# argmaxinc/DiffusionKit

Measured on NVIDIA H100. Metric: images/sec at 1024x1024 (FLUX.1-schnell 4-step), higher is better.
Workload: dtype bf16

## Files before the change

### diffusionkit_b200/build.py

```python
import os
import subprocess
import sys

HERE = os.path.dirname(os.path.abspath(__file__))
CSRC = os.path.join(HERE, "csrc")
LIB = os.path.join(HERE, "libdkb200.so")
SOURCES = ["api.cu", "gemm.cu", "conv_fused.cu", "attention.cu", "elementwise.cu", "text.cu"]
NVCC_FLAGS = [
    "-gencode", "arch=compute_90a,code=sm_90a",
    "-O3", "-lineinfo", "-std=c++17",
    "-Xcompiler", "-fPIC", "-Xcompiler", "-Wall",
    "--expt-relaxed-constexpr",
    "-Xptxas", "-v",
]


def _stale(obj, src):
    if not os.path.exists(obj):
        return True
    t = os.path.getmtime(obj)
    deps = [src] + [os.path.join(CSRC, f) for f in os.listdir(CSRC) if f.endswith((".cuh", ".h"))]
    deps.append(os.path.join(HERE, "..", "include", "dkb200.h"))
    return any(os.path.getmtime(d) > t for d in deps)


def build(force: bool = False, verbose: bool = False) -> str:
    nvcc = os.environ.get("NVCC", "/usr/local/cuda/bin/nvcc")
    objs = []
    procs = []
    for s in SOURCES:
        src = os.path.join(CSRC, s)
        if not os.path.exists(src):
            continue
        obj = os.path.join(CSRC, s.replace(".cu", ".o"))
        objs.append(obj)
        if force or _stale(obj, src):
            cmd = [nvcc, *NVCC_FLAGS, "-c", src, "-o", obj]
            procs.append((s, subprocess.Popen(cmd, stdout=subprocess.PIPE, stderr=subprocess.STDOUT, text=True)))
    failed = False
    for s, p in procs:
        out, _ = p.communicate()
        if p.returncode != 0:
            failed = True
            sys.stderr.write(f"[build] {s} FAILED\n{out}\n")
        elif verbose:
            sys.stderr.write(f"[build] {s}\n{out}\n")
    if failed:
        raise RuntimeError("nvcc failed")
    if procs or not os.path.exists(LIB):
        cmd = [nvcc, "-shared", "-Wno-deprecated-gpu-targets", "-o", LIB, *objs, "-lcudart", "-ldl"]
        subprocess.check_call(cmd)
    return LIB


if __name__ == "__main__":
    print(build(force="--force" in sys.argv, verbose="-v" in sys.argv))
```

### diffusionkit_b200/csrc/attention.cu

```cuda
#include "attention.cuh"

namespace dk {

constexpr int ATT_THREADS = 384;

template <typename T, int D>
__global__ void __launch_bounds__(ATT_THREADS, 1)
attention_fwd_kernel(const __grid_constant__ CUtensorMap tm, const AttParams p) {
  using H16 = Half16<T>;
  using Cfg = AttCfg<D>;
  constexpr int KS = Cfg::KS;
  extern __shared__ uint8_t smem_raw[];
  uint8_t* smem = smem_raw + ((1024u - (smem_u32(smem_raw) & 1023u)) & 1023u);
  uint8_t* sQ = smem + Cfg::OFF_Q;
  uint8_t* sK = smem + Cfg::OFF_K;
  uint8_t* sV = smem + Cfg::OFF_V;
  uint64_t* q_full = reinterpret_cast<uint64_t*>(smem + Cfg::OFF_BAR);
  uint64_t* k_full = q_full + 1;
  uint64_t* v_full = k_full + KS;
  uint64_t* kv_empty = v_full + KS;

  const int warp = threadIdx.x >> 5;
  const int lane = threadIdx.x & 31;
  const int wg = threadIdx.x >> 7;
  const int q0 = blockIdx.x * ATT_BQ;
  const int head = blockIdx.y;
  const int b = blockIdx.z;
  const int h = p.heads * D;
  const int row0 = b * p.S;
  const int nkv = (p.S + ATT_BKV - 1) / ATT_BKV;
  constexpr uint32_t TILE_BYTES = ATT_BKV * D * 2;

  if (threadIdx.x == 0) {
    tma_prefetch_desc(&tm);
    mbar_init(q_full, 1);
    for (int i = 0; i < KS; ++i) {
      mbar_init(&k_full[i], 1);
      mbar_init(&v_full[i], 1);
      mbar_init(&kv_empty[i], 8);
    }
    fence_barrier_init();
  }
  __syncthreads();

  if (wg == 0) {
    if (warp != 0) return;
    if (elect_one_sync()) {
      mbar_arrive_expect_tx(q_full, ATT_BQ * D * 2);
#pragma unroll
      for (int c = 0; c < D / 64; ++c) tma_load_2d(sQ + c * (ATT_BQ * 128), &tm, q_full, head * D + c * 64, row0 + q0);
    }
    __syncwarp();
    uint32_t stage = 0, phase = 0;
    for (int j = 0; j < nkv; ++j) {
      mbar_wait_warp(&kv_empty[stage], phase ^ 1);
      if (elect_one_sync()) {
        const int kr = row0 + j * ATT_BKV;
        mbar_arrive_expect_tx(&k_full[stage], TILE_BYTES);
#pragma unroll
        for (int c = 0; c < D / 64; ++c)
          tma_load_2d(sK + stage * TILE_BYTES + c * (ATT_BKV * 128), &tm, &k_full[stage], h + head * D + c * 64, kr);
        mbar_arrive_expect_tx(&v_full[stage], TILE_BYTES);
#pragma unroll
        for (int c = 0; c < D / 64; ++c)
          tma_load_2d(sV + stage * TILE_BYTES + c * (ATT_BKV * 128), &tm, &v_full[stage], 2 * h + head * D + c * 64, kr);
      }
      __syncwarp();
      if (++stage == KS) {
        stage = 0;
        phase ^= 1;
      }
    }
    return;
  }

  const int cw = wg - 1;
  const float sl2 = p.scale_log2;
  float o[D / 2];
#pragma unroll
  for (int i = 0; i < D / 2; ++i) o[i] = 0.f;
  float m_run[2] = {-INFINITY, -INFINITY};
  float l_run[2] = {0.f, 0.f};
  const int col0 = 2 * (lane & 3);

  mbar_wait(q_full, 0);
  const uint32_t q_base = smem_u32(sQ) + cw * 64 * 128;
  uint32_t stage = 0, phase = 0;
  for (int j = 0; j < nkv; ++j) {
    const int kv_valid = p.S - j * ATT_BKV;
    const uint32_t k_base = smem_u32(sK + stage * TILE_BYTES);
    const uint32_t v_base = smem_u32(sV + stage * TILE_BYTES);
    float s[ATT_BKV / 2];
    mbar_wait(&k_full[stage], phase);
    wgmma_fence();
#pragma unroll
    for (int kk = 0; kk < D / 16; ++kk) {
      const uint32_t koff = (kk >> 2) * (ATT_BKV * 128) + (kk & 3) * 32;
      Wgmma<ATT_BKV, H16::is_bf16, 0>::ss(s, make_smem_desc_sw128(q_base + (kk >> 2) * (ATT_BQ * 128) + (kk & 3) * 32, 16, 1024),
                                         make_smem_desc_sw128(k_base + koff, 16, 1024), kk != 0 ? 1u : 0u);
    }
    wgmma_commit();
    wgmma_wait<0>();
    reg_fence(s);

    float alpha[2];
#pragma unroll
    for (int i = 0; i < 2; ++i) {
      float mx = -INFINITY;
#pragma unroll
      for (int jj = 0; jj < ATT_BKV / 8; ++jj)
#pragma unroll
        for (int e = 0; e < 2; ++e) {
          float& v = s[4 * jj + 2 * i + e];
          if (kv_valid < ATT_BKV && 8 * jj + col0 + e >= kv_valid) v = -INFINITY;
          mx = fmaxf(mx, v);
        }
      mx = fmaxf(mx, __shfl_xor_sync(0xffffffffu, mx, 1));
      mx = fmaxf(mx, __shfl_xor_sync(0xffffffffu, mx, 2));
      const float m_new = fmaxf(m_run[i], mx * sl2);
      alpha[i] = ex2_approx(m_run[i] - m_new);
      m_run[i] = m_new;
      float ls = 0.f;
#pragma unroll
      for (int jj = 0; jj < ATT_BKV / 8; ++jj)
#pragma unroll
        for (int e = 0; e < 2; ++e) {
          float& v = s[4 * jj + 2 * i + e];
          v = ex2_approx(fmaf(v, sl2, -m_new));
          ls += v;
        }
      l_run[i] = l_run[i] * alpha[i] + ls;
    }
#pragma unroll
    for (int jj = 0; jj < D / 8; ++jj)
#pragma unroll
      for (int i = 0; i < 2; ++i) {
        o[4 * jj + 2 * i] *= alpha[i];
        o[4 * jj + 2 * i + 1] *= alpha[i];
      }
    uint32_t pa[ATT_BKV / 16][4];
#pragma unroll
    for (int kk = 0; kk < ATT_BKV / 16; ++kk) {
      pa[kk][0] = H16::pack(s[8 * kk + 0], s[8 * kk + 1]);
      pa[kk][1] = H16::pack(s[8 * kk + 2], s[8 * kk + 3]);
      pa[kk][2] = H16::pack(s[8 * kk + 4], s[8 * kk + 5]);
      pa[kk][3] = H16::pack(s[8 * kk + 6], s[8 * kk + 7]);
    }

    mbar_wait(&v_full[stage], phase);
    wgmma_fence();
#pragma unroll
    for (int kk = 0; kk < ATT_BKV / 16; ++kk)
      Wgmma<D, H16::is_bf16, 1>::rs(o, pa[kk], make_smem_desc_sw128(v_base + kk * 16 * 128, ATT_BKV * 128, 1024), 1u);
    wgmma_commit();
    wgmma_wait<0>();
    reg_fence(o);
    __syncwarp();
    if (lane == 0) mbar_arrive(&kv_empty[stage]);
    if (++stage == KS) {
      stage = 0;
      phase ^= 1;
    }
  }

#pragma unroll
  for (int i = 0; i < 2; ++i) {
    float l = l_run[i];
    l += __shfl_xor_sync(0xffffffffu, l, 1);
    l += __shfl_xor_sync(0xffffffffu, l, 2);
    const float inv_l = 1.0f / l;
    const int s_idx = q0 + cw * 64 + (warp & 3) * 16 + (lane >> 2) + 8 * i;
    if (s_idx >= p.S) continue;
    T* dst;
    if (s_idx < p.split)
      dst = reinterpret_cast<T*>(p.out0) + (static_cast<long long>(b) * p.split + s_idx) * p.ld0 + head * D;
    else
      dst = reinterpret_cast<T*>(p.out1) + (static_cast<long long>(b) * (p.S - p.split) + (s_idx - p.split)) * p.ld1 +
            head * D;
#pragma unroll
    for (int jj = 0; jj < D / 8; ++jj)
      *reinterpret_cast<uint32_t*>(dst + 8 * jj + col0) =
          H16::pack(o[4 * jj + 2 * i] * inv_l, o[4 * jj + 2 * i + 1] * inv_l);
  }
}

template <typename T, int D>
static int launch_attention(dk_ctx* ctx, const CUtensorMap& tm, const AttParams& p, cudaStream_t stream) {
  auto kern = attention_fwd_kernel<T, D>;
  static bool configured = false;
  if (!configured) {
    DK_CHECK_CUDA(cudaFuncSetAttribute(kern, cudaFuncAttributeMaxDynamicSharedMemorySize, AttCfg<D>::SMEM_BYTES));
    configured = true;
  }
  dim3 grid(dk_ceil_div(p.S, ATT_BQ), p.heads, p.B);
  kern<<<grid, ATT_THREADS, AttCfg<D>::SMEM_BYTES, stream>>>(tm, p);
  DK_LAUNCH_CHECK(ctx);
  return 0;
}

}

using namespace dk;

extern "C" int dk_attention_fwd(dk_ctx* ctx, int dtype, const void* qkv, int B, int S, int heads, int d, float scale,
                                int split, void* out0, long long ld0, void* out1, long long ld1, void* stream_) {
  DK_REQUIRE(ctx != nullptr, "dk_attention_fwd: null ctx");
  DkDeviceGuard dk_guard_(ctx);
  DK_REQUIRE(dtype == DK_BF16 || dtype == DK_FP16, "dk_attention_fwd: bad dtype %d", dtype);
  DK_REQUIRE(d == 64 || d == 128, "dk_attention_fwd: head dim %d unsupported (64 or 128)", d);
  DK_REQUIRE(B > 0 && S > 0 && heads > 0, "dk_attention_fwd: empty problem");
  DK_REQUIRE(split >= 0 && split <= S, "dk_attention_fwd: split %d outside [0, %d]", split, S);
  DK_REQUIRE(out0 != nullptr || split == 0, "dk_attention_fwd: out0 is NULL");
  DK_REQUIRE(out1 != nullptr || split == S, "dk_attention_fwd: out1 is NULL but split < S");
  DK_REQUIRE(ld0 % 8 == 0 && ld1 % 8 == 0, "dk_attention_fwd: output leading dims must be multiples of 8");
  DK_REQUIRE((reinterpret_cast<uintptr_t>(qkv) & 15u) == 0 && (reinterpret_cast<uintptr_t>(out0) & 15u) == 0 &&
                 (reinterpret_cast<uintptr_t>(out1) & 15u) == 0,
             "dk_attention_fwd: buffers must be 16-byte aligned");
  cudaStream_t stream = static_cast<cudaStream_t>(stream_);
  const int h = heads * d;
  CUtensorMap tm;
  const uint64_t dims[2] = {static_cast<uint64_t>(3 * h), static_cast<uint64_t>(B) * S};
  const uint64_t strides[1] = {static_cast<uint64_t>(3 * h) * 2};
  const uint32_t box[2] = {64, 128};
  if (int rc = dk_make_tmap_16b(ctx, &tm, qkv, 2, dims, strides, box)) return rc;
  AttParams p;
  p.B = B;
  p.S = S;
  p.heads = heads;
  p.split = split;
  p.scale_log2 = scale * 1.44269504088896341f;
  p.out0 = out0;
  p.ld0 = ld0;
  p.out1 = out1;
  p.ld1 = ld1;
  if (dtype == DK_BF16) {
    if (d == 128) return launch_attention<__nv_bfloat16, 128>(ctx, tm, p, stream);
    return launch_attention<__nv_bfloat16, 64>(ctx, tm, p, stream);
  }
  if (d == 128) return launch_attention<__half, 128>(ctx, tm, p, stream);
  return launch_attention<__half, 64>(ctx, tm, p, stream);
}
```

### diffusionkit_b200/csrc/common.cuh

```cuda
#pragma once

#include <cuda.h>
#include <cuda_bf16.h>
#include <cuda_fp16.h>
#include <cuda_runtime.h>
#include <stdint.h>
#include <stdio.h>

#include "wgmma.cuh"

namespace dk {

__device__ __forceinline__ uint32_t smem_u32(const void* p) {
  return static_cast<uint32_t>(__cvta_generic_to_shared(p));
}


#ifndef DK_WATCHDOG_CYCLES
#define DK_WATCHDOG_CYCLES (8000000000LL)
#endif

__device__ __forceinline__ void mbar_init(uint64_t* bar, uint32_t count) {
  asm volatile("mbarrier.init.shared::cta.b64 [%0], %1;" ::"r"(smem_u32(bar)), "r"(count) : "memory");
}
__device__ __forceinline__ void fence_barrier_init() {
  asm volatile("fence.mbarrier_init.release.cluster;" ::: "memory");
}
__device__ __forceinline__ void mbar_arrive(uint64_t* bar) {
  asm volatile("mbarrier.arrive.shared::cta.b64 _, [%0];" ::"r"(smem_u32(bar)) : "memory");
}
__device__ __forceinline__ void mbar_arrive_expect_tx(uint64_t* bar, uint32_t bytes) {
  asm volatile("mbarrier.arrive.expect_tx.shared::cta.b64 _, [%0], %1;" ::"r"(smem_u32(bar)), "r"(bytes)
               : "memory");
}
__device__ __forceinline__ uint32_t mbar_try_wait(uint64_t* bar, uint32_t parity) {
  uint32_t ok;
  asm volatile(
      "{\n\t.reg .pred p;\n\t"
      "mbarrier.try_wait.parity.shared::cta.b64 p, [%1], %2;\n\t"
      "selp.u32 %0, 1, 0, p;\n\t}"
      : "=r"(ok)
      : "r"(smem_u32(bar)), "r"(parity)
      : "memory");
  return ok;
}
#ifndef DK_WATCHDOG_SPINS
#define DK_WATCHDOG_SPINS (1u << 26)
#endif
static __device__ __noinline__ void mbar_watchdog_trap(uint64_t* bar, uint32_t parity) {
  printf("[dkb200] mbarrier watchdog: block (%d,%d,%d) thread %d bar@%u parity %u\n", blockIdx.x, blockIdx.y, blockIdx.z,
         threadIdx.x, smem_u32(bar), parity);
  __trap();
}
__device__ __forceinline__ void mbar_wait(uint64_t* bar, uint32_t parity) {
  if (mbar_try_wait(bar, parity)) return;
  uint32_t spins = 0;
  while (!mbar_try_wait(bar, parity)) {
    if (++spins == DK_WATCHDOG_SPINS) mbar_watchdog_trap(bar, parity);
  }
}

__device__ __forceinline__ void mbar_wait_nocall(uint64_t* bar, uint32_t parity) {
  uint32_t spins = 0;
  while (!mbar_try_wait(bar, parity)) {
    if (++spins == DK_WATCHDOG_SPINS) asm volatile("trap;");
  }
}

__device__ __forceinline__ void mbar_wait_warp(uint64_t* bar, uint32_t parity) {
  if ((threadIdx.x & 31) == 0) mbar_wait(bar, parity);
  __syncwarp();
}

__device__ __forceinline__ void st_shared_u32(uint32_t addr, uint32_t v) {
  asm volatile("st.shared.u32 [%0], %1;" ::"r"(addr), "r"(v));
}

__device__ __forceinline__ void fence_proxy_async_smem() {
  asm volatile("fence.proxy.async.shared::cta;" ::: "memory");
}

__device__ __forceinline__ void named_bar_sync(uint32_t id, uint32_t nthreads) {
  asm volatile("bar.sync %0, %1;" ::"r"(id), "r"(nthreads) : "memory");
}

__device__ __forceinline__ uint32_t cluster_ctarank() {
  uint32_t r;
  asm volatile("mov.u32 %0, %%cluster_ctarank;" : "=r"(r));
  return r;
}
__device__ __forceinline__ void cluster_sync() {
  asm volatile("barrier.cluster.arrive.release;\n\tbarrier.cluster.wait.acquire;" ::: "memory");
}
__device__ __forceinline__ void mbar_arrive_cluster(uint64_t* bar, uint32_t cta) {
  asm volatile(
      "{\n\t.reg .b32 ra;\n\t"
      "mapa.shared::cluster.u32 ra, %0, %1;\n\t"
      "mbarrier.arrive.shared::cluster.b64 _, [ra];\n\t}" ::"r"(smem_u32(bar)),
      "r"(cta)
      : "memory");
}

__device__ __forceinline__ void tma_prefetch_desc(const CUtensorMap* m) {
  asm volatile("prefetch.tensormap [%0];" ::"l"(reinterpret_cast<uint64_t>(m)) : "memory");
}
__device__ __forceinline__ void tma_load_2d(void* dst, const CUtensorMap* map, uint64_t* bar, int c0, int c1) {
  asm volatile(
      "cp.async.bulk.tensor.2d.shared::cluster.global.tile.mbarrier::complete_tx::bytes [%0], [%1, {%3, %4}], [%2];" ::
          "r"(smem_u32(dst)),
      "l"(reinterpret_cast<uint64_t>(map)), "r"(smem_u32(bar)), "r"(c0), "r"(c1)
      : "memory");
}
__device__ __forceinline__ void tma_load_2d_multicast(void* dst, const CUtensorMap* map, uint64_t* bar, int c0, int c1,
                                                      uint16_t cta_mask) {
  asm volatile(
      "cp.async.bulk.tensor.2d.shared::cluster.global.tile.mbarrier::complete_tx::bytes.multicast::cluster "
      "[%0], [%1, {%3, %4}], [%2], %5;" ::"r"(smem_u32(dst)),
      "l"(reinterpret_cast<uint64_t>(map)), "r"(smem_u32(bar)), "r"(c0), "r"(c1), "h"(cta_mask)
      : "memory");
}
__device__ __forceinline__ void tma_load_4d(void* dst, const CUtensorMap* map, uint64_t* bar, int c0, int c1, int c2,
                                            int c3) {
  asm volatile(
      "cp.async.bulk.tensor.4d.shared::cluster.global.tile.mbarrier::complete_tx::bytes [%0], [%1, {%3, %4, %5, %6}], "
      "[%2];" ::"r"(smem_u32(dst)),
      "l"(reinterpret_cast<uint64_t>(map)), "r"(smem_u32(bar)), "r"(c0), "r"(c1), "r"(c2), "r"(c3)
      : "memory");
}

__device__ __forceinline__ void wgmma_fence() { asm volatile("wgmma.fence.sync.aligned;" ::: "memory"); }
__device__ __forceinline__ void wgmma_commit() { asm volatile("wgmma.commit_group.sync.aligned;" ::: "memory"); }
template <int N>
__device__ __forceinline__ void wgmma_wait() {
  asm volatile("wgmma.wait_group.sync.aligned %0;" ::"n"(N) : "memory");
}
template <int N>
__device__ __forceinline__ void reg_fence(float (&d)[N]) {
#pragma unroll
  for (int i = 0; i < N; ++i) asm volatile("" : "+f"(d[i])::"memory");
}

template <int N>
__device__ __forceinline__ void setmaxnreg_inc() {
  asm volatile("setmaxnreg.inc.sync.aligned.u32 %0;" ::"n"(N));
}
template <int N>
__device__ __forceinline__ void setmaxnreg_dec() {
  asm volatile("setmaxnreg.dec.sync.aligned.u32 %0;" ::"n"(N));
}
__device__ __forceinline__ float ex2_approx(float x) {
  float y;
  asm("ex2.approx.ftz.f32 %0, %1;" : "=f"(y) : "f"(x));
  return y;
}

__device__ __forceinline__ uint64_t make_smem_desc_sw128(uint32_t smem_addr, uint32_t lbo_bytes, uint32_t sbo_bytes) {
  uint64_t d = 0;
  d |= static_cast<uint64_t>((smem_addr & 0x3FFFFu) >> 4);
  d |= static_cast<uint64_t>((lbo_bytes >> 4) & 0x3FFFu) << 16;
  d |= static_cast<uint64_t>((sbo_bytes >> 4) & 0x3FFFu) << 32;
  d |= static_cast<uint64_t>(1) << 62;
  return d;
}

__device__ __forceinline__ bool elect_one_sync() {
  uint32_t pred;
  asm volatile(
      "{\n\t.reg .pred p;\n\t"
      "elect.sync _|p, 0xffffffff;\n\t"
      "selp.u32 %0, 1, 0, p;\n\t}"
      : "=r"(pred));
  return pred != 0;
}

template <int N>
__device__ __forceinline__ void stage_acc_rows(float* stage, int ld, int row0, const float (&d)[N / 2]) {
  const int t = threadIdx.x & 127;
  const int r = row0 + (t >> 5) * 16 + ((t & 31) >> 2);
  const int c = 2 * (t & 3);
#pragma unroll
  for (int j = 0; j < N / 8; ++j)
#pragma unroll
    for (int i = 0; i < 2; ++i)
      *reinterpret_cast<float2*>(stage + (r + 8 * i) * ld + 8 * j + c) = make_float2(d[4 * j + 2 * i], d[4 * j + 2 * i + 1]);
}

template <typename T>
struct Half16;
template <>
struct Half16<__nv_bfloat16> {
  using T2 = __nv_bfloat162;
  static constexpr bool is_bf16 = true;
  __device__ static __forceinline__ float to_f(__nv_bfloat16 v) { return __bfloat162float(v); }
  __device__ static __forceinline__ __nv_bfloat16 from_f(float v) { return __float2bfloat16_rn(v); }
  __device__ static __forceinline__ uint32_t pack(float lo, float hi) {
    __nv_bfloat162 t = __floats2bfloat162_rn(lo, hi);
    return *reinterpret_cast<uint32_t*>(&t);
  }
  __device__ static __forceinline__ float2 unpack(uint32_t u) {
    __nv_bfloat162 t = *reinterpret_cast<__nv_bfloat162*>(&u);
    return __bfloat1622float2(t);
  }
};
template <>
struct Half16<__half> {
  using T2 = __half2;
  static constexpr bool is_bf16 = false;
  __device__ static __forceinline__ float to_f(__half v) { return __half2float(v); }
  __device__ static __forceinline__ __half from_f(float v) { return __float2half_rn(v); }
  __device__ static __forceinline__ uint32_t pack(float lo, float hi) {
    __half2 t = __floats2half2_rn(lo, hi);
    return *reinterpret_cast<uint32_t*>(&t);
  }
  __device__ static __forceinline__ float2 unpack(uint32_t u) {
    __half2 t = *reinterpret_cast<__half2*>(&u);
    return __half22float2(t);
  }
};

__device__ __forceinline__ float gelu_erf(float v) { return 0.5f * v * (1.0f + erff(v * 0.70710678118654752f)); }
__device__ __forceinline__ float silu_f(float v) {
  float e;
  asm("ex2.approx.ftz.f32 %0, %1;" : "=f"(e) : "f"(-1.4426950408889634f * v));
  return __fdividef(v, 1.0f + e);
}

__device__ __forceinline__ float quick_gelu_f(float v) {
  float e;
  asm("ex2.approx.ftz.f32 %0, %1;" : "=f"(e) : "f"(-1.702f * 1.4426950408889634f * v));
  return __fdividef(v, 1.0f + e);
}

__device__ __forceinline__ float warp_sum(float v) {
#pragma unroll
  for (int o = 16; o > 0; o >>= 1) v += __shfl_xor_sync(0xffffffffu, v, o);
  return v;
}
__device__ __forceinline__ float warp_max(float v) {
#pragma unroll
  for (int o = 16; o > 0; o >>= 1) v = fmaxf(v, __shfl_xor_sync(0xffffffffu, v, o));
  return v;
}

}
```

### diffusionkit_b200/csrc/conv_fused.cu

```cuda
#include <stdlib.h>

#include "common.cuh"
#include "host.h"

namespace dk {

constexpr int CF_TW = 128;
constexpr int CF_R = 2;
constexpr int CF_BN = 128;
constexpr int CF_HW = CF_TW + 2;
constexpr int CF_HR = CF_R + 2;
constexpr int CF_A_BYTES = CF_HR * CF_HW * 128;
constexpr int CF_B_BYTES = CF_BN * 64 * 2;
constexpr int CF_A_BUFS = 2;
constexpr int CF_B_STAGES = 4;
constexpr int CF_THREADS = 384;
constexpr int CF_STAGE_LD = CF_BN + 4;
constexpr int CF_STAT_BYTES = 8 * CF_R * 2 * 8 * 2 * 4;
constexpr int CF_OFF_B = CF_A_BUFS * CF_A_BYTES;
constexpr int CF_OFF_STAT = CF_OFF_B + CF_B_STAGES * CF_B_BYTES;
constexpr int CF_OFF_BAR = CF_OFF_STAT + CF_STAT_BYTES;
constexpr int CF_SMEM_BYTES = CF_OFF_BAR + 256 + 1024;
static_assert(CF_OFF_STAT >= CF_R * CF_TW * CF_STAGE_LD * 4, "conv_fused: the staging tile reuses the pipeline buffers");
static_assert(CF_SMEM_BYTES <= 232448, "conv_fused: shared memory budget");

struct ConvFParams {
  int B, H, W;
  int Cin, Cout;
  int up;
  int tiles_x, tiles_y;
  int n_tiles;
  const void* bias;
  const void* res;
  void* out;
  const float* gn_stats;
  const void* gamma;
  const void* beta;
  int G;
  int silu;
  float* out_partial;
  int out_G;
};

__device__ __forceinline__ float tanh_approx(float x) {
  float y;
  asm("tanh.approx.f32 %0, %1;" : "=f"(y) : "f"(x));
  return y;
}

struct CfItem {
  int b, ty, tx, phase, nt;
};
__device__ __forceinline__ void cf_decode(const ConvFParams& p, int item, CfItem& it) {
  const int phases = p.up ? 4 : 1;
  it.nt = item % p.n_tiles;
  item /= p.n_tiles;
  it.phase = item % phases;
  item /= phases;
  it.tx = item % p.tiles_x;
  item /= p.tiles_x;
  it.ty = item % p.tiles_y;
  it.b = item / p.tiles_y;
}

template <int N>
__device__ __forceinline__ void warp_multi_sum(float (&v)[N], int lane) {
  int off = 16;
#pragma unroll
  for (int n = N; n > 1; n >>= 1, off >>= 1) {
    const bool hi = (lane & off) != 0;
#pragma unroll
    for (int i = 0; i < n / 2; ++i) {
      const float keep = hi ? v[i + n / 2] : v[i];
      const float send = hi ? v[i] : v[i + n / 2];
      v[i] = keep + __shfl_xor_sync(0xffffffffu, send, off);
    }
  }
#pragma unroll
  for (; off > 0; off >>= 1) v[0] += __shfl_xor_sync(0xffffffffu, v[0], off);
}
template <int N>
__device__ __forceinline__ int warp_multi_index(int lane) {
  int idx = 0, off = 16;
#pragma unroll
  for (int n = N; n > 1; n >>= 1, off >>= 1) idx += (lane & off) ? n / 2 : 0;
  return idx;
}

template <int CPG>
__device__ __forceinline__ void cf_chunk_stats(const float (&v)[32], float* dst, int lane) {
  constexpr int NG = 32 / CPG;
  constexpr int N = 2 * NG;
  float a[N];
#pragma unroll
  for (int g = 0; g < NG; ++g) {
    float s = 0.f, q = 0.f;
#pragma unroll
    for (int c = 0; c < CPG; ++c) {
      const float t = v[g * CPG + c];
      s += t;
      q = fmaf(t, t, q);
    }
    a[g] = s;
    a[NG + g] = q;
  }
  warp_multi_sum<N>(a, lane);
  constexpr int LOW = 32 / N;
  if ((lane & (LOW - 1)) == 0) {
    const int idx = warp_multi_index<N>(lane);
    const int g = idx % NG, which = idx / NG;
    dst[g * 2 + which] = a[0];
  }
}

template <typename T>
__global__ void __launch_bounds__(CF_THREADS, 1)
conv_fused_kernel(const __grid_constant__ CUtensorMap tmX, const __grid_constant__ CUtensorMap tmW, const ConvFParams p) {
  using H16 = Half16<T>;
  extern __shared__ uint8_t smem_raw[];
  uint8_t* smem = smem_raw + ((1024u - (smem_u32(smem_raw) & 1023u)) & 1023u);
  uint8_t* sA = smem;
  uint8_t* sB = smem + CF_OFF_B;
  float* sstat = reinterpret_cast<float*>(smem + CF_OFF_STAT);
  uint64_t* bars = reinterpret_cast<uint64_t*>(smem + CF_OFF_BAR);
  uint64_t* a_land = bars;
  uint64_t* a_empty = a_land + CF_A_BUFS;
  uint64_t* b_full = a_empty + CF_A_BUFS;
  uint64_t* b_empty = b_full + CF_B_STAGES;

  const int warp = threadIdx.x >> 5;
  const int lane = threadIdx.x & 31;
  const int wg = threadIdx.x >> 7;
  const int cblocks = p.Cin / 64;
  const int ntaps = p.up ? 4 : 9;
  CfItem it;
  cf_decode(p, blockIdx.x, it);
  const int py = it.phase >> 1, px = it.phase & 1;
  const int y0 = it.ty * CF_R;
  const int x0 = it.tx * CF_TW;

  if (threadIdx.x == 0) {
    tma_prefetch_desc(&tmX);
    tma_prefetch_desc(&tmW);
    for (int i = 0; i < CF_A_BUFS; ++i) {
      mbar_init(&a_land[i], 1);
      mbar_init(&a_empty[i], 8);
    }
    for (int i = 0; i < CF_B_STAGES; ++i) {
      mbar_init(&b_full[i], 1);
      mbar_init(&b_empty[i], 8);
    }
    fence_barrier_init();
  }
  __syncthreads();

  if (wg == 0) {
    if (warp != 0) return;
    uint32_t bst = 0, bph = 0;
    uint32_t abuf = 0, aph = 0;
    const int w_row = it.phase * p.Cout + it.nt * CF_BN;
    for (int cb = 0; cb < cblocks; ++cb) {
      mbar_wait_warp(&a_empty[abuf], aph ^ 1);
      if (elect_one_sync()) {
        mbar_arrive_expect_tx(&a_land[abuf], CF_A_BYTES);
        tma_load_4d(sA + abuf * CF_A_BYTES, &tmX, &a_land[abuf], cb * 64, x0 - 1, y0 - 1, it.b);
      }
      __syncwarp();
      if (++abuf == CF_A_BUFS) {
        abuf = 0;
        aph ^= 1;
      }
      for (int tap = 0; tap < ntaps; ++tap) {
        mbar_wait_warp(&b_empty[bst], bph ^ 1);
        if (elect_one_sync()) {
          mbar_arrive_expect_tx(&b_full[bst], CF_B_BYTES);
          tma_load_2d(sB + bst * CF_B_BYTES, &tmW, &b_full[bst], tap * p.Cin + cb * 64, w_row);
        }
        __syncwarp();
        if (++bst == CF_B_STAGES) {
          bst = 0;
          bph ^= 1;
        }
      }
    }
    return;
  }

  const int rr = wg - 1;
  const int tid = threadIdx.x - 128;
  float acc0[CF_BN / 2], acc1[CF_BN / 2];
#pragma unroll
  for (int i = 0; i < CF_BN / 2; ++i) {
    acc0[i] = 0.f;
    acc1[i] = 0.f;
  }
  {
    constexpr int TT = 256;
    const int chunk = tid & 7;
    const int cpg = p.gn_stats != nullptr ? p.Cin / p.G : 1;
    uint32_t bst = 0, bph = 0, abuf = 0, aph = 0;
    for (int cb = 0; cb < cblocks; ++cb) {
      mbar_wait(&a_land[abuf], aph);
      if (p.gn_stats != nullptr) {
        float sc[8], sh[8];
        {
          const int c0 = cb * 64 + chunk * 8;
          const uint4 g4 = *reinterpret_cast<const uint4*>(reinterpret_cast<const T*>(p.gamma) + c0);
          const uint4 b4 = *reinterpret_cast<const uint4*>(reinterpret_cast<const T*>(p.beta) + c0);
          const uint32_t gw[4] = {g4.x, g4.y, g4.z, g4.w}, bw[4] = {b4.x, b4.y, b4.z, b4.w};
#pragma unroll
          for (int i = 0; i < 4; ++i) {
            const float2 gf = H16::unpack(gw[i]), bf = H16::unpack(bw[i]);
#pragma unroll
            for (int h2 = 0; h2 < 2; ++h2) {
              const int g = (c0 + 2 * i + h2) / cpg;
              const float mean = __ldg(p.gn_stats + (it.b * p.G + g) * 2), rstd = __ldg(p.gn_stats + (it.b * p.G + g) * 2 + 1);
              const float ga = h2 ? gf.y : gf.x, be = h2 ? bf.y : bf.x;
              sc[2 * i + h2] = rstd * ga;
              sh[2 * i + h2] = be - mean * rstd * ga;
            }
          }
        }
        const uint32_t base = smem_u32(sA) + abuf * CF_A_BYTES;
        const bool do_silu = p.silu != 0;
        auto in_image = [&](int q) {
          const int hr = q / CF_HW, hx = q - hr * CF_HW;
          const int gy = y0 - 1 + hr, gx = x0 - 1 + hx;
          return q < CF_HR * CF_HW && gy >= 0 && gy < p.H && gx >= 0 && gx < p.W;
        };
        auto xform = [&](uint32_t (&w)[4]) {
#pragma unroll
          for (int i = 0; i < 4; ++i) {
            const float2 f = H16::unpack(w[i]);
            float a = fmaf(f.x, sc[2 * i], sh[2 * i]);
            float b = fmaf(f.y, sc[2 * i + 1], sh[2 * i + 1]);
            if (do_silu) {
              const float ha = 0.5f * a, hb = 0.5f * b;
              a = fmaf(ha, tanh_approx(ha), ha);
              b = fmaf(hb, tanh_approx(hb), hb);
            }
            w[i] = H16::pack(a, b);
          }
        };
        for (int q0 = tid >> 3; q0 < CF_HR * CF_HW; q0 += 2 * (TT / 8)) {
          const int q1 = q0 + TT / 8;
          const bool ok0 = in_image(q0), ok1 = in_image(q1);
          const uint32_t addr0 = base + q0 * 128 + ((chunk ^ (q0 & 7)) << 4);
          const uint32_t addr1 = base + q1 * 128 + ((chunk ^ (q1 & 7)) << 4);
          uint32_t w0[4] = {0u, 0u, 0u, 0u}, w1[4] = {0u, 0u, 0u, 0u};
          if (ok0) asm volatile("ld.shared.v4.b32 {%0, %1, %2, %3}, [%4];" : "=r"(w0[0]), "=r"(w0[1]), "=r"(w0[2]), "=r"(w0[3]) : "r"(addr0));
          if (ok1) asm volatile("ld.shared.v4.b32 {%0, %1, %2, %3}, [%4];" : "=r"(w1[0]), "=r"(w1[1]), "=r"(w1[2]), "=r"(w1[3]) : "r"(addr1));
          xform(w0);
          xform(w1);
          if (ok0) asm volatile("st.shared.v4.b32 [%0], {%1, %2, %3, %4};" ::"r"(addr0), "r"(w0[0]), "r"(w0[1]), "r"(w0[2]), "r"(w0[3]) : "memory");
          if (ok1) asm volatile("st.shared.v4.b32 [%0], {%1, %2, %3, %4};" ::"r"(addr1), "r"(w1[0]), "r"(w1[1]), "r"(w1[2]), "r"(w1[3]) : "memory");
        }
        fence_proxy_async_smem();
        named_bar_sync(1, 256);
      }
      const uint32_t a_addr0 = smem_u32(sA) + abuf * CF_A_BYTES;
      uint32_t prev = 0;
      for (int tap = 0; tap < ntaps; ++tap) {
        const int dy = p.up ? ((tap >> 1) + py) : (tap / 3);
        const int dx = p.up ? ((tap & 1) + px) : (tap - (tap / 3) * 3);
        mbar_wait(&b_full[bst], bph);
        const uint32_t b_addr = smem_u32(sB) + bst * CF_B_BYTES;
        const uint32_t a_addr = a_addr0 + ((rr + dy) * CF_HW + dx) * 128;
        wgmma_fence();
#pragma unroll
        for (int k = 0; k < 4; ++k) {
          const uint32_t acc_on = (cb | tap | k) != 0 ? 1u : 0u;
          const uint64_t db = make_smem_desc_sw128(b_addr + k * 32, 16, 1024);
          Wgmma<CF_BN, H16::is_bf16, 0>::ss(acc0, make_smem_desc_sw128(a_addr + k * 32, 16, 1024), db, acc_on);
          Wgmma<CF_BN, H16::is_bf16, 0>::ss(acc1, make_smem_desc_sw128(a_addr + 64 * 128 + k * 32, 16, 1024), db, acc_on);
        }
        wgmma_commit();
        if (tap > 0) {
          wgmma_wait<1>();
          if (lane == 0) mbar_arrive(&b_empty[prev]);
        }
        prev = bst;
        if (++bst == CF_B_STAGES) {
          bst = 0;
          bph ^= 1;
        }
      }
      wgmma_wait<0>();
      if (lane == 0) {
        mbar_arrive(&b_empty[prev]);
        mbar_arrive(&a_empty[abuf]);
      }
      if (++abuf == CF_A_BUFS) {
        abuf = 0;
        aph ^= 1;
      }
    }
    reg_fence(acc0);
    reg_fence(acc1);
  }

  float* stg = reinterpret_cast<float*>(smem);
  named_bar_sync(1, 256);
  stage_acc_rows<CF_BN>(stg, CF_STAGE_LD, rr * CF_TW, acc0);
  stage_acc_rows<CF_BN>(stg, CF_STAGE_LD, rr * CF_TW + 64, acc1);
  named_bar_sync(1, 256);

  const int ew = warp - 4;
  const int quarter = ew & 3;
  const int half = ew >> 2;
  const int xl = quarter * 32 + lane;
  const T* bias = reinterpret_cast<const T*>(p.bias);
  const T* res = reinterpret_cast<const T*>(p.res);
  T* out = reinterpret_cast<T*>(p.out);
  const int Hout = p.up ? 2 * p.H : p.H, Wout = p.up ? 2 * p.W : p.W;
  const int cpg_out = p.out_partial != nullptr ? p.Cout / p.out_G : 8;
  const int slots = (Hout * Wout) / CF_TW;
  const int x = x0 + xl;
  const int n_base = it.nt * CF_BN + half * 64;
  float* st_my = sstat + (ew * CF_R) * (2 * 8 * 2);
#pragma unroll 1
  for (int r2 = 0; r2 < CF_R; ++r2) {
    const int oy = p.up ? 2 * (y0 + r2) + py : (y0 + r2);
    const int ox = p.up ? 2 * x + px : x;
    const long long orow = (static_cast<long long>(it.b) * Hout + oy) * Wout + ox;
#pragma unroll
    for (int ch = 0; ch < 2; ++ch) {
      const float* src = stg + (r2 * CF_TW + xl) * CF_STAGE_LD + half * 64 + ch * 32;
      const int n0 = n_base + ch * 32;
      float v[32];
#pragma unroll
      for (int j = 0; j < 4; ++j) {
        if (n0 + j * 8 >= p.Cout) {
#pragma unroll
          for (int i = 0; i < 8; ++i) v[j * 8 + i] = 0.f;
          continue;
        }
        const float4 a4 = *reinterpret_cast<const float4*>(src + j * 8);
        const float4 b4f = *reinterpret_cast<const float4*>(src + j * 8 + 4);
        const float r[8] = {a4.x, a4.y, a4.z, a4.w, b4f.x, b4f.y, b4f.z, b4f.w};
        float bv[8] = {0.f, 0.f, 0.f, 0.f, 0.f, 0.f, 0.f, 0.f};
        if (bias != nullptr) {
          const uint4 b4 = *reinterpret_cast<const uint4*>(bias + n0 + j * 8);
          const uint32_t bw[4] = {b4.x, b4.y, b4.z, b4.w};
#pragma unroll
          for (int i = 0; i < 4; ++i) {
            const float2 f = H16::unpack(bw[i]);
            bv[2 * i] = f.x;
            bv[2 * i + 1] = f.y;
          }
        }
        float rv[8] = {0.f, 0.f, 0.f, 0.f, 0.f, 0.f, 0.f, 0.f};
        if (res != nullptr) {
          const uint4 r4 = *reinterpret_cast<const uint4*>(res + orow * p.Cout + n0 + j * 8);
          const uint32_t rw[4] = {r4.x, r4.y, r4.z, r4.w};
#pragma unroll
          for (int i = 0; i < 4; ++i) {
            const float2 f = H16::unpack(rw[i]);
            rv[2 * i] = f.x;
            rv[2 * i + 1] = f.y;
          }
        }
        uint32_t w16[4];
#pragma unroll
        for (int i = 0; i < 4; ++i) {
          const float a = r[2 * i] + bv[2 * i] + rv[2 * i];
          const float b = r[2 * i + 1] + bv[2 * i + 1] + rv[2 * i + 1];
          w16[i] = H16::pack(a, b);
          const float2 back = H16::unpack(w16[i]);
          v[j * 8 + 2 * i] = back.x;
          v[j * 8 + 2 * i + 1] = back.y;
        }
        *reinterpret_cast<uint4*>(out + orow * p.Cout + n0 + j * 8) = make_uint4(w16[0], w16[1], w16[2], w16[3]);
      }
      if (p.out_partial != nullptr) {
        float* dst = st_my + ((r2 * 2 + ch) * 8) * 2;
        if (cpg_out == 4)
          cf_chunk_stats<4>(v, dst, lane);
        else if (cpg_out == 8)
          cf_chunk_stats<8>(v, dst, lane);
        else
          cf_chunk_stats<16>(v, dst, lane);
      }
    }
  }
  if (p.out_partial != nullptr) {
    named_bar_sync(1, 256);
    const int ng = 32 / cpg_out;
    const int per_row = 2 * 2 * ng;
    if (tid < CF_R * per_row) {
      const int r2 = tid / per_row;
      const int rem = tid - r2 * per_row;
      const int hf = rem / (2 * ng);
      const int ch = (rem / ng) & 1;
      const int g = rem % ng;
      float s = 0.f, q = 0.f;
#pragma unroll
      for (int qd = 0; qd < 4; ++qd) {
        const float* src = sstat + ((hf * 4 + qd) * CF_R) * (2 * 8 * 2) + ((r2 * 2 + ch) * 8 + g) * 2;
        s += src[0];
        q += src[1];
      }
      const int oy = p.up ? 2 * (y0 + r2) + py : (y0 + r2);
      const int slot = p.up ? ((oy * p.tiles_x + it.tx) * 2 + px) : (oy * p.tiles_x + it.tx);
      const int gidx = (it.nt * CF_BN + hf * 64 + ch * 32) / cpg_out + g;
      float* dst = p.out_partial + ((static_cast<long long>(it.b) * slots + slot) * p.out_G + gidx) * 2;
      dst[0] = s;
      dst[1] = q;
    }
  }
}

template <typename T>
__global__ void conv_up_weights_kernel(const T* __restrict__ w, T* __restrict__ wp, int Cout, int Cin) {
  const long long total = 4LL * Cout * 4 * Cin;
  for (long long i = blockIdx.x * static_cast<long long>(blockDim.x) + threadIdx.x; i < total;
       i += static_cast<long long>(gridDim.x) * blockDim.x) {
    const int c = static_cast<int>(i % Cin);
    long long t = i / Cin;
    const int tap = static_cast<int>(t % 4);
    t /= 4;
    const int n = static_cast<int>(t % Cout);
    const int phase = static_cast<int>(t / Cout);
    const int py = phase >> 1, px = phase & 1, a = tap >> 1, b = tap & 1;
    const int ky0 = (py == 0) ? (a == 0 ? 0 : 1) : (a == 0 ? 0 : 2);
    const int ky1 = (py == 0) ? (a == 0 ? 0 : 2) : (a == 0 ? 1 : 2);
    const int kx0 = (px == 0) ? (b == 0 ? 0 : 1) : (b == 0 ? 0 : 2);
    const int kx1 = (px == 0) ? (b == 0 ? 0 : 2) : (b == 0 ? 1 : 2);
    float acc = 0.f;
    for (int ky = ky0; ky <= ky1; ++ky)
      for (int kx = kx0; kx <= kx1; ++kx) acc += Half16<T>::to_f(w[((static_cast<long long>(n) * 3 + ky) * 3 + kx) * Cin + c]);
    wp[i] = Half16<T>::from_f(acc);
  }
}

}

using namespace dk;

static bool cf_aligned16(const void* p) { return (reinterpret_cast<uintptr_t>(p) & 15u) == 0; }

extern "C" int dk_conv_fused_supported(int H, int W, int Cin, int Cout) {
  const bool cout_ok = Cout % CF_BN == 0 || (Cout > 0 && Cout < CF_BN && Cout % 8 == 0);
  return (W % CF_TW == 0 && H % (2 * CF_R) == 0 && Cin % 64 == 0 && Cin <= 512 && cout_ok) ? 1 : 0;
}

extern "C" int dk_conv_up_weights(dk_ctx* ctx, int dtype, const void* w, void* wp, int Cout, int Cin, void* stream_) {
  DK_REQUIRE(ctx != nullptr, "dk_conv_up_weights: null ctx");
  DkDeviceGuard dk_guard_(ctx);
  DK_REQUIRE(dtype == DK_BF16 || dtype == DK_FP16, "dk_conv_up_weights: bad dtype %d", dtype);
  DK_REQUIRE(w != nullptr && wp != nullptr && Cout > 0 && Cin > 0, "dk_conv_up_weights: bad arguments");
  cudaStream_t stream = static_cast<cudaStream_t>(stream_);
  const long long total = 16LL * Cout * Cin;
  const int grid = static_cast<int>((total + 255) / 256 < 4096 ? (total + 255) / 256 : 4096);
  if (dtype == DK_BF16)
    conv_up_weights_kernel<__nv_bfloat16><<<grid, 256, 0, stream>>>(static_cast<const __nv_bfloat16*>(w),
                                                                      static_cast<__nv_bfloat16*>(wp), Cout, Cin);
  else
    conv_up_weights_kernel<__half><<<grid, 256, 0, stream>>>(static_cast<const __half*>(w), static_cast<__half*>(wp), Cout, Cin);
  DK_LAUNCH_CHECK(ctx);
  return 0;
}

extern "C" int dk_conv3x3_fused(dk_ctx* ctx, int dtype, const void* x, const void* w, const void* bias, const void* res,
                                void* out, int B, int H, int W, int Cin, int Cout, int up, const float* gn_stats,
                                const void* gamma, const void* beta, int G, int silu, float* out_partial, int out_G,
                                void* stream_) {
  DK_REQUIRE(ctx != nullptr, "dk_conv3x3_fused: null ctx");
  DkDeviceGuard dk_guard_(ctx);
  DK_REQUIRE(dtype == DK_BF16 || dtype == DK_FP16, "dk_conv3x3_fused: bad dtype %d", dtype);
  DK_REQUIRE(B > 0 && dk_conv_fused_supported(H, W, Cin, Cout),
             "dk_conv3x3_fused: needs W %% 128 == 0, H %% 4 == 0, Cin %% 64 == 0 (<= 512), Cout %% 128 == 0 or a multiple "
             "of 8 below 128 (got %dx%d, %d -> %d)",
             H, W, Cin, Cout);
  DK_REQUIRE(Cout % CF_BN == 0 || (up == 0 && out_partial == nullptr),
             "dk_conv3x3_fused: a narrow output tile (Cout = %d) has no upsampling and no output statistics", Cout);
  DK_REQUIRE(cf_aligned16(x) && cf_aligned16(w) && cf_aligned16(out) && (bias == nullptr || cf_aligned16(bias)) &&
                 (res == nullptr || cf_aligned16(res)),
             "dk_conv3x3_fused: buffers must be 16-byte aligned");
  DK_REQUIRE(gn_stats == nullptr || (gamma != nullptr && beta != nullptr && G > 0 && Cin % G == 0),
             "dk_conv3x3_fused: GroupNorm needs gamma, beta and G dividing Cin");
  DK_REQUIRE(gn_stats == nullptr || up == 0, "dk_conv3x3_fused: normalisation and upsampling are not combined");
  DK_REQUIRE(out_partial == nullptr || (out_G > 0 && Cout % out_G == 0 && (Cout / out_G == 4 || Cout / out_G == 8 || Cout / out_G == 16)),
             "dk_conv3x3_fused: output statistics need 4, 8 or 16 channels per group");
  cudaStream_t stream = static_cast<cudaStream_t>(stream_);
  ConvFParams p = {};
  p.B = B;
  p.H = H;
  p.W = W;
  p.Cin = Cin;
  p.Cout = Cout;
  p.up = up ? 1 : 0;
  p.tiles_x = W / CF_TW;
  p.tiles_y = H / CF_R;
  p.n_tiles = (Cout + CF_BN - 1) / CF_BN;
  p.bias = bias;
  p.res = res;
  p.out = out;
  p.gn_stats = gn_stats;
  p.gamma = gamma;
  p.beta = beta;
  p.G = G;
  p.silu = silu;
  p.out_partial = out_partial;
  p.out_G = out_G;

  CUtensorMap tmX, tmW;
  {
    const uint64_t dims[4] = {static_cast<uint64_t>(Cin), static_cast<uint64_t>(W), static_cast<uint64_t>(H),
                              static_cast<uint64_t>(B)};
    const uint64_t strides[3] = {static_cast<uint64_t>(Cin) * 2, static_cast<uint64_t>(W) * Cin * 2,
                                 static_cast<uint64_t>(H) * W * Cin * 2};
    const uint32_t box[4] = {64, CF_HW, CF_HR, 1};
    if (int rc = dk_make_tmap_16b(ctx, &tmX, x, 4, dims, strides, box)) return rc;
  }
  {
    const int taps = up ? 4 : 9;
    const uint64_t dims[2] = {static_cast<uint64_t>(taps) * Cin, static_cast<uint64_t>(up ? 4 : 1) * Cout};
    const uint64_t strides[1] = {static_cast<uint64_t>(taps) * Cin * 2};
    const uint32_t box[2] = {64, CF_BN};
    if (int rc = dk_make_tmap_16b(ctx, &tmW, w, 2, dims, strides, box)) return rc;
  }
  const long long items = static_cast<long long>(B) * p.tiles_y * p.tiles_x * (up ? 4 : 1) * p.n_tiles;
  DK_REQUIRE(items < (1LL << 31), "dk_conv3x3_fused: problem too large");
  if (dtype == DK_BF16) {
    auto kern = conv_fused_kernel<__nv_bfloat16>;
    static bool configured = false;
    if (!configured) {
      DK_CHECK_CUDA(cudaFuncSetAttribute(kern, cudaFuncAttributeMaxDynamicSharedMemorySize, CF_SMEM_BYTES));
      configured = true;
    }
    kern<<<static_cast<int>(items), CF_THREADS, CF_SMEM_BYTES, stream>>>(tmX, tmW, p);
  } else {
    auto kern = conv_fused_kernel<__half>;
    static bool configured = false;
    if (!configured) {
      DK_CHECK_CUDA(cudaFuncSetAttribute(kern, cudaFuncAttributeMaxDynamicSharedMemorySize, CF_SMEM_BYTES));
      configured = true;
    }
    kern<<<static_cast<int>(items), CF_THREADS, CF_SMEM_BYTES, stream>>>(tmX, tmW, p);
  }
  DK_LAUNCH_CHECK(ctx);
  return 0;
}
```

Before: 1.370.

## Ping-pong attention consumer warpgroups and drop noinline watchdog from mbarrier waits

The two consumer warpgroups in the attention kernel now take turns through named barriers, so one warpgroup's QK^T wgmma can overlap the other's softmax, FA3-style ping-pong scheduling. The mbar_wait helper, which called a noinline printf/trap routine, is removed and every call site uses the inline wait variant. This is meant to stop ptxas from serialising wgmma instructions because of the function call. The build now fails if ptxas reports serialised wgmma. The turn-taking adds barrier traffic and could deadlock if the arrive/sync counts are unbalanced.

```diff
diff --git a/diffusionkit_b200/build.py b/diffusionkit_b200/build.py
--- a/diffusionkit_b200/build.py
+++ b/diffusionkit_b200/build.py
@@ -13,6 +13,7 @@
     "--expt-relaxed-constexpr",
     "-Xptxas", "-v",
 ]
+SERIALISED_WGMMA = "wgmma.mma_async instructions are serialized"
 
 
 def _stale(obj, src):
@@ -43,6 +44,10 @@
         if p.returncode != 0:
             failed = True
             sys.stderr.write(f"[build] {s} FAILED\n{out}\n")
+        elif SERIALISED_WGMMA in out:
+            failed = True
+            os.remove(os.path.join(CSRC, s.replace(".cu", ".o")))
+            sys.stderr.write(f"[build] {s} FAILED: ptxas serialised its wgmma instructions\n{out}\n")
         elif verbose:
             sys.stderr.write(f"[build] {s}\n{out}\n")
     if failed:
diff --git a/diffusionkit_b200/csrc/attention.cu b/diffusionkit_b200/csrc/attention.cu
--- a/diffusionkit_b200/csrc/attention.cu
+++ b/diffusionkit_b200/csrc/attention.cu
@@ -3,6 +3,7 @@
 namespace dk {
 
 constexpr int ATT_THREADS = 384;
+constexpr uint32_t ATT_TURN_BAR = 1;
 
 template <typename T, int D>
 __global__ void __launch_bounds__(ATT_THREADS, 1)
@@ -83,15 +84,19 @@
   float l_run[2] = {0.f, 0.f};
   const int col0 = 2 * (lane & 3);
 
-  mbar_wait(q_full, 0);
+  const uint32_t turn_mine = ATT_TURN_BAR + cw, turn_other = ATT_TURN_BAR + (cw ^ 1);
+  if (cw == 1) named_bar_arrive(turn_other, 256);
+
+  mbar_wait_nocall(q_full, 0);
   const uint32_t q_base = smem_u32(sQ) + cw * 64 * 128;
   uint32_t stage = 0, phase = 0;
+  named_bar_sync(turn_mine, 256);
   for (int j = 0; j < nkv; ++j) {
     const int kv_valid = p.S - j * ATT_BKV;
     const uint32_t k_base = smem_u32(sK + stage * TILE_BYTES);
     const uint32_t v_base = smem_u32(sV + stage * TILE_BYTES);
     float s[ATT_BKV / 2];
-    mbar_wait(&k_full[stage], phase);
+    mbar_wait_nocall(&k_full[stage], phase);
     wgmma_fence();
 #pragma unroll
     for (int kk = 0; kk < D / 16; ++kk) {
@@ -100,6 +105,7 @@
                                          make_smem_desc_sw128(k_base + koff, 16, 1024), kk != 0 ? 1u : 0u);
     }
     wgmma_commit();
+    named_bar_arrive(turn_other, 256);
     wgmma_wait<0>();
     reg_fence(s);
 
@@ -147,7 +153,8 @@
       pa[kk][3] = H16::pack(s[8 * kk + 6], s[8 * kk + 7]);
     }
 
-    mbar_wait(&v_full[stage], phase);
+    mbar_wait_nocall(&v_full[stage], phase);
+    named_bar_sync(turn_mine, 256);
     wgmma_fence();
 #pragma unroll
     for (int kk = 0; kk < ATT_BKV / 16; ++kk)
@@ -162,6 +169,7 @@
       phase ^= 1;
     }
   }
+  if (cw == 0) named_bar_arrive(turn_other, 256);
 
 #pragma unroll
   for (int i = 0; i < 2; ++i) {
diff --git a/diffusionkit_b200/csrc/common.cuh b/diffusionkit_b200/csrc/common.cuh
--- a/diffusionkit_b200/csrc/common.cuh
+++ b/diffusionkit_b200/csrc/common.cuh
@@ -47,19 +47,6 @@
 #ifndef DK_WATCHDOG_SPINS
 #define DK_WATCHDOG_SPINS (1u << 26)
 #endif
-static __device__ __noinline__ void mbar_watchdog_trap(uint64_t* bar, uint32_t parity) {
-  printf("[dkb200] mbarrier watchdog: block (%d,%d,%d) thread %d bar@%u parity %u\n", blockIdx.x, blockIdx.y, blockIdx.z,
-         threadIdx.x, smem_u32(bar), parity);
-  __trap();
-}
-__device__ __forceinline__ void mbar_wait(uint64_t* bar, uint32_t parity) {
-  if (mbar_try_wait(bar, parity)) return;
-  uint32_t spins = 0;
-  while (!mbar_try_wait(bar, parity)) {
-    if (++spins == DK_WATCHDOG_SPINS) mbar_watchdog_trap(bar, parity);
-  }
-}
-
 __device__ __forceinline__ void mbar_wait_nocall(uint64_t* bar, uint32_t parity) {
   uint32_t spins = 0;
   while (!mbar_try_wait(bar, parity)) {
@@ -68,7 +55,7 @@
 }
 
 __device__ __forceinline__ void mbar_wait_warp(uint64_t* bar, uint32_t parity) {
-  if ((threadIdx.x & 31) == 0) mbar_wait(bar, parity);
+  if ((threadIdx.x & 31) == 0) mbar_wait_nocall(bar, parity);
   __syncwarp();
 }
 
@@ -82,6 +69,9 @@
 
 __device__ __forceinline__ void named_bar_sync(uint32_t id, uint32_t nthreads) {
   asm volatile("bar.sync %0, %1;" ::"r"(id), "r"(nthreads) : "memory");
+}
+__device__ __forceinline__ void named_bar_arrive(uint32_t id, uint32_t nthreads) {
+  asm volatile("bar.arrive %0, %1;" ::"r"(id), "r"(nthreads) : "memory");
 }
 
 __device__ __forceinline__ uint32_t cluster_ctarank() {
diff --git a/diffusionkit_b200/csrc/conv_fused.cu b/diffusionkit_b200/csrc/conv_fused.cu
--- a/diffusionkit_b200/csrc/conv_fused.cu
+++ b/diffusionkit_b200/csrc/conv_fused.cu
@@ -200,7 +200,7 @@
     const int cpg = p.gn_stats != nullptr ? p.Cin / p.G : 1;
     uint32_t bst = 0, bph = 0, abuf = 0, aph = 0;
     for (int cb = 0; cb < cblocks; ++cb) {
-      mbar_wait(&a_land[abuf], aph);
+      mbar_wait_nocall(&a_land[abuf], aph);
       if (p.gn_stats != nullptr) {
         float sc[8], sh[8];
         {
@@ -263,7 +263,7 @@
       for (int tap = 0; tap < ntaps; ++tap) {
         const int dy = p.up ? ((tap >> 1) + py) : (tap / 3);
         const int dx = p.up ? ((tap & 1) + px) : (tap - (tap / 3) * 3);
-        mbar_wait(&b_full[bst], bph);
+        mbar_wait_nocall(&b_full[bst], bph);
         const uint32_t b_addr = smem_u32(sB) + bst * CF_B_BYTES;
         const uint32_t a_addr = a_addr0 + ((rr + dy) * CF_HW + dx) * 128;
         wgmma_fence();
```

Measured after the change: 1.431 (median of 6 runs). +4.5%, better.
